# kongqg/marl-sat

Measured on AMD Instinct MI355X. Metric: env-steps/sec (whole node) + MAPPO updates/sec, 4096 envs random 3-SAT, higher is better.
Workload: dtype int32

## Files before the change

marl-sat_amd/csrc/env_kernels.hip:

```cpp
#include <stdlib.h>

#include <algorithm>

#include "common.h"
#include "obs_sparse.h"

namespace msat {

constexpr int kThreads = 256;

struct EnvParams {
    int B, V, C, K, A, M, D;
    int WV, WC;
    int base, rem;
    int max_steps, action_mode, reward_mode, N;
    float r_clause, r_sat, gamma;
    int ablate;
    long long dbg_obs, dbg_assign, dbg_sat, dbg_ntrue, dbg_actions;
    int rq_mode, rq_cap;
    uint32_t rq_serial;
};

struct ObsShadowArg {
    uint32_t *rows;
    int g;
};

enum : int { kModeReset = 0, kModeStep = 1, kModeStepAutoReset = 2, kModeObs = 3 };

__host__ __device__ __forceinline__ uint32_t rq_token(uint32_t serial) { return 0x80000000u | (serial & 0x7FFFFFFFu); }
__host__ __device__ __forceinline__ int rq_capacity(int B) { return (B / 256 + 8 + 7) & ~7; }
__host__ __device__ __forceinline__ size_t rq_words(int B) { return 2 * (size_t)B; }

__device__ __forceinline__ uint32_t *rq_pend(uint32_t *q, int B, int par) { return q + (size_t)par * B; }

__device__ __forceinline__ int rq_scan(const uint32_t *__restrict__ pend, int B, uint32_t tok, int lim, int want,
                                       int *sel) {
    const int lane = threadIdx.x & 63;
    const int W = ((B + 63) / 64 + 3) & ~3;
    const int lo = lane * W;
    int below = 0, mine = 0;
    uint64_t bits = 0;
    for (int i = 0; i < W; i += 4) {
        const int k = lo + i;
        uint4 v = make_uint4(0u, 0u, 0u, 0u);
        if (k < B) v = *reinterpret_cast<const uint4 *>(pend + k);
        const uint32_t w[4] = {v.x, v.y, v.z, v.w};
#pragma unroll
        for (int u = 0; u < 4; ++u) {
            const bool m = k + u < B && w[u] == tok;
            mine += m;
            below += m && k + u < lim;
            if (m && i + u < 64) bits |= 1ull << (i + u);
        }
    }
    int total_below = below;
#pragma unroll
    for (int d = 32; d >= 1; d >>= 1) total_below += __shfl_xor(total_below, d, 64);
    if (want >= 0) {
        int incl = mine;
#pragma unroll
        for (int d = 1; d < 64; d <<= 1) {
            const int up = __shfl_up(incl, d, 64);
            if (lane >= d) incl += up;
        }
        const int excl = incl - mine;
        int found = -1;
        if (want >= excl && want < incl) {
            int r = want - excl;
            if (W <= 64) {
                uint64_t m = bits;
                for (; r > 0; --r) m &= m - 1;
                found = lo + __ffsll((unsigned long long)m) - 1;
            } else {
                for (int i = 0; i < W && found < 0; i += 4) {
                    const int k = lo + i;
                    if (k >= B) break;
                    const uint4 v = *reinterpret_cast<const uint4 *>(pend + k);
                    const uint32_t w[4] = {v.x, v.y, v.z, v.w};
                    for (int u = 0; u < 4 && found < 0; ++u)
                        if (k + u < B && w[u] == tok && r-- == 0) found = k + u;
                }
            }
        }
        const uint64_t has = __ballot(found >= 0);
        *sel = has ? __shfl(found, __ffsll((unsigned long long)has) - 1, 64) : -1;
    }
    return total_below;
}

__host__ __device__ __forceinline__ int agent_lo(const EnvParams &p, int i) { return i * p.base + (i < p.rem ? i : p.rem); }
__host__ __device__ __forceinline__ int agent_size(const EnvParams &p, int i) { return p.base + (i < p.rem ? 1 : 0); }

__device__ __forceinline__ int agent_of_var(const EnvParams &p, int v) {
    const int split = p.rem * (p.base + 1);
    if (v < split) return v / (p.base + 1);
    return p.rem + (v - split) / p.base;
}

struct EnvLds {
    uint32_t *x;
    uint32_t *sat;
    uint32_t *rel;
    uint32_t *nbr;
    uint32_t *fm;
    uint32_t *fx;
    int *red;
    uint32_t *fd;
    uint32_t *sx;
    uint32_t *ssat;
};

__host__ __device__ __forceinline__ int obs_image_words(const EnvParams &p) { return (p.A * p.D) / 32 + 2; }

__host__ __device__ __forceinline__ int shadow_row_words(const EnvParams &p) {
    return 1 + ((p.V + 31) >> 5) + ((p.C + 31) >> 5);
}

__host__ __device__ __forceinline__ size_t env_lds_words(const EnvParams &p, bool sh = false) {
    return (size_t)p.WV + p.WC + (size_t)p.A * (p.WC + p.WV) + 2 * (size_t)obs_image_words(p) + 16 +
           (sh ? (size_t)obs_image_words(p) + 1 + p.WV + p.WC : 0);
}

template <bool SH = false>
__device__ __forceinline__ EnvLds carve(uint32_t *smem, const EnvParams &p) {
    EnvLds l;
    l.x = smem;
    l.sat = l.x + p.WV;
    l.rel = l.sat + p.WC;
    l.nbr = l.rel + (size_t)p.A * p.WC;
    l.fm = l.nbr + (size_t)p.A * p.WV;
    l.fx = l.fm + obs_image_words(p);
    l.fd = l.fx + obs_image_words(p);
    l.sx = l.fd + (SH ? obs_image_words(p) + 1 : 0);
    l.ssat = l.sx + (SH ? p.WV : 0);
    l.red = reinterpret_cast<int *>(l.ssat + (SH ? p.WC : 0));
    return l;
}

__device__ __forceinline__ uint32_t bit(const uint32_t *w, int i) { return (w[i >> 5] >> (i & 31)) & 1u; }

template <int T>
__device__ __forceinline__ void load_x_bits(const EnvParams &p, const EnvLds &l, const uint8_t *__restrict__ xg,
                                            uint32_t x0) {
    const int lane = threadIdx.x & 63;
    for (int v0 = threadIdx.x & ~63; v0 < p.WV * 32; v0 += T) {
        const int v = v0 + lane;
        const uint32_t xv = v0 == (int)(threadIdx.x & ~63) ? x0 : (v < p.V ? xg[v] : 0u);
        const uint64_t m = __ballot(v < p.V && (xv & 1u));
        if (lane < 2) l.x[(v0 >> 5) + lane] = (uint32_t)(m >> (32 * lane));
    }
}
template <int T>
__device__ __forceinline__ void load_x_bits(const EnvParams &p, const EnvLds &l, const uint8_t *__restrict__ xg) {
    load_x_bits<T>(p, l, xg, (int)threadIdx.x < p.V ? xg[threadIdx.x] : 0u);
}

constexpr int kPfClause = 4;
constexpr int kPfRel = 4;
constexpr int kPfNbr = 2;

template <bool kPbrs>
__device__ __forceinline__ void clause_slice(const EnvParams &p, const EnvLds &l, int c0, uint64_t w,
                                             uint8_t *__restrict__ sat_g, uint8_t *__restrict__ ntrue_g, int &unsat,
                                             int &newly) {
    const int lane = threadIdx.x & 63;
    const int c = c0 + lane;
    uint32_t sat = 0, ntrue = 0, old = 0;
    const bool live = c < p.C;
    if (live) {
#pragma unroll
        for (int j = 0; j < 3; ++j) {
            const uint32_t lit = (uint32_t)(w >> (16 * j)) & 0xFFFFu;
            if (lit < MSAT_LIT_ABSENT) ntrue += (bit(l.x, (int)(lit >> 1)) ^ lit) & 1u;
        }
        sat = ntrue ? 1u : 0u;
        if (kPbrs) old = sat_g[c];
        if (sat_g) sat_g[c] = (uint8_t)sat;
        if (ntrue_g) ntrue_g[c] = (uint8_t)ntrue;
    }
    const uint64_t ms = __ballot(sat);
    if (lane < 2) l.sat[(c0 >> 5) + lane] = (uint32_t)(ms >> (32 * lane));
    unsat += __popcll(__ballot(live && !sat));
    if (kPbrs) newly += __popcll(__ballot(sat && !old));
}

template <int T, bool kPbrs, int NPF>
__device__ __forceinline__ void eval_clauses(const EnvParams &p, const EnvLds &l, const uint16_t *__restrict__ lits,
                                             int pidx, uint8_t *__restrict__ sat_g, uint8_t *__restrict__ ntrue_g,
                                             const uint64_t (&pw)[kPfClause]) {
    const uint64_t *prow = reinterpret_cast<const uint64_t *>(lits) + (size_t)pidx * p.C;
    const int lane = threadIdx.x & 63;
    int unsat = 0, newly = 0;
    const int cend = p.WC * 32;
#pragma unroll
    for (int j = 0; j < NPF; ++j) {
        const int c0 = (threadIdx.x & ~63) + j * T;
        if (c0 < cend) clause_slice<kPbrs>(p, l, c0, pw[j], sat_g, ntrue_g, unsat, newly);
    }
    for (int c0 = (threadIdx.x & ~63) + NPF * T; c0 < cend; c0 += T) {
        const int c = c0 + lane;
        const uint64_t w = c < p.C ? prow[c] : 0ull;
        clause_slice<kPbrs>(p, l, c0, w, sat_g, ntrue_g, unsat, newly);
    }
    if (lane == 0) {
        atomicAdd(&l.red[0], unsat);
        if (kPbrs) atomicAdd(&l.red[1], newly);
    }
}


__device__ __forceinline__ uint32_t low_mask(int n) { return n >= 32 ? 0xFFFFFFFFu : ((1u << n) - 1u); }

__device__ __forceinline__ void or_bits(uint32_t *img, int dst, uint32_t bits) {
    if (!bits) return;
    const int w = dst >> 5, s = dst & 31;
    atomicOr(&img[w], bits << s);
    if (s) {
        const uint32_t hi = bits >> (32 - s);
        if (hi) atomicOr(&img[w + 1], hi);
    }
}

template <int T, bool SH>
__device__ __forceinline__ void build_obs_images(const EnvParams &p, const EnvLds &l, bool delta) {
    const int nwV = (p.V + 31) >> 5, nwC = (p.C + 31) >> 5;
    const int U = 2 * nwV + nwC;
    for (int t = threadIdx.x; t < p.A * U; t += T) {
        const int i = t / U;
        int s = t - i * U;
        int len, off;
        uint32_t m, x, xo = 0;
        if (s < nwV) {
            len = min(32, p.V - 32 * s);
            const int lo = agent_lo(p, i) - 32 * s, hi = lo + agent_size(p, i);
            const int a = max(lo, 0), z = min(hi, 32);
            m = z > a ? (low_mask(z) & ~low_mask(a)) : 0u;
            x = l.x[s];
            if (SH && delta) xo = l.sx[s];
            off = 32 * s;
        } else if ((s -= nwV) < nwC) {
            len = min(32, p.C - 32 * s);
            m = l.rel[i * p.WC + s];
            x = l.sat[s];
            if (SH && delta) xo = l.ssat[s];
            off = p.V + 32 * s;
        } else {
            s -= nwC;
            len = min(32, p.V - 32 * s);
            m = l.nbr[i * p.WV + s];
            x = l.x[s];
            if (SH && delta) xo = l.sx[s];
            off = p.V + p.C + 32 * s;
        }
        const uint32_t keep = low_mask(len);
        const int dst = i * p.D + off;
        or_bits(l.fm, dst, m & keep);
        or_bits(l.fx, dst, x & m & keep);
        if (SH && delta) or_bits(l.fd, dst, (x ^ xo) & m & keep);
    }
}

__device__ __forceinline__ uint32_t bits_at(const uint32_t *img, int e) {
    const int w = e >> 5, s = e & 31;
    return (uint32_t)((((uint64_t)img[w + 1] << 32) | img[w]) >> s);
}

__device__ __forceinline__ int elem_val(uint32_t m, uint32_t x, int u) {
    return ((m >> u) & 1u) ? (int)((x >> u) & 1u) : -1;
}

template <typename ObsT>
struct ObsVec;
template <>
struct ObsVec<int32_t> {
    static constexpr int N = 4;
    __device__ static void store(int32_t *dst, uint32_t m, uint32_t x) {
        typedef int v4i __attribute__((ext_vector_type(4)));
        const v4i q = {elem_val(m, x, 0), elem_val(m, x, 1), elem_val(m, x, 2), elem_val(m, x, 3)};
        *reinterpret_cast<v4i *>(dst) = q;
    }
};
template <>
struct ObsVec<int8_t> {
    static constexpr int N = 16;
    __device__ static void store(int8_t *dst, uint32_t m, uint32_t x) {
        typedef unsigned v4u __attribute__((ext_vector_type(4)));
        v4u q;
#pragma unroll
        for (int w = 0; w < 4; ++w) {
            uint32_t word = 0;
#pragma unroll
            for (int u = 0; u < 4; ++u) word |= ((uint32_t)elem_val(m, x, 4 * w + u) & 0xFFu) << (8 * u);
            q[w] = word;
        }
        *reinterpret_cast<v4u *>(dst) = q;
    }
};

template <int T, typename ObsT>
__device__ __forceinline__ void write_obs(const EnvParams &p, const EnvLds &l, ObsT *__restrict__ o) {
    constexpr int VEC = ObsVec<ObsT>::N;
    const int total = p.A * p.D;
    int head = (int)((reinterpret_cast<uintptr_t>(o) / sizeof(ObsT)) % VEC);
    head = head ? VEC - head : 0;
    head = min(head, total);
    for (int e = threadIdx.x; e < head; e += T) o[e] = (ObsT)elem_val(bits_at(l.fm, e), bits_at(l.fx, e), 0);
    const int nchunks = (total - head) / VEC;
    for (int q = threadIdx.x; q < nchunks; q += T) {
        const int e = head + q * VEC;
        ObsVec<ObsT>::store(o + e, bits_at(l.fm, e), bits_at(l.fx, e));
    }
    for (int e = head + nchunks * VEC + threadIdx.x; e < total; e += T)
        o[e] = (ObsT)elem_val(bits_at(l.fm, e), bits_at(l.fx, e), 0);
}

template <typename ObsT>
__device__ __forceinline__ void dcheck_obs_kept(const EnvLds &l, const ObsT *o, int e, int n) {
#ifdef MSAT_DEBUG
    for (int u = 0; u < n; ++u)
        MSAT_DCHECK((int)o[e + u] == elem_val(bits_at(l.fm, e + u), bits_at(l.fx, e + u), 0) ? 0 : -1 - (e + u), 1);
#endif
}

template <int T, typename ObsT>
__device__ __forceinline__ void write_obs_delta(const EnvParams &p, const EnvLds &l, ObsT *__restrict__ o, int G) {
    constexpr int VEC = ObsVec<ObsT>::N;
    const int total = p.A * p.D;
    const uintptr_t a0 = reinterpret_cast<uintptr_t>(o) / sizeof(ObsT);
    const int GE = G / (int)sizeof(ObsT);
    int head = (int)(a0 % VEC);
    head = head ? VEC - head : 0;
    head = min(head, total);
    for (int e = threadIdx.x; e < head; e += T) {
        if (bit(l.fd, e))
            o[e] = (ObsT)elem_val(bits_at(l.fm, e), bits_at(l.fx, e), 0);
        else
            dcheck_obs_kept(l, o, e, 1);
    }
    const int nchunks = (total - head) / VEC;
    for (int q = threadIdx.x; q < nchunks; q += T) {
        const int e = head + q * VEC;
        const int gs = e - (int)((a0 + (uintptr_t)e) & (uintptr_t)(GE - 1));
        const int lo = max(gs, 0), hi = min(gs + GE, total);
        uint32_t any = 0;
        for (int k = lo; k < hi; k += 32) any |= bits_at(l.fd, k) & low_mask(hi - k);
        if (any)
            ObsVec<ObsT>::store(o + e, bits_at(l.fm, e), bits_at(l.fx, e));
        else
            dcheck_obs_kept(l, o, e, VEC);
    }
    for (int e = head + nchunks * VEC + threadIdx.x; e < total; e += T) {
        if (bit(l.fd, e))
            o[e] = (ObsT)elem_val(bits_at(l.fm, e), bits_at(l.fx, e), 0);
        else
            dcheck_obs_kept(l, o, e, 1);
    }
}

__device__ __forceinline__ int xcd_major(int blk, int n, bool off) {
    return (!off && (n & 7) == 0) ? (blk & 7) * (n >> 3) + (blk >> 3) : blk;
}

__device__ __forceinline__ void lds_barrier() { asm volatile("s_waitcnt lgkmcnt(0)\n\ts_barrier" ::: "memory"); }

struct ClockStamp {
    uint64_t *buf = nullptr;
    uint64_t t0 = 0, r0 = 0;
    __device__ __forceinline__ ClockStamp(uint64_t *stamps, int b) {
        if (stamps != nullptr) {
            t0 = __builtin_amdgcn_s_memtime();
            r0 = __builtin_amdgcn_s_memrealtime();
            buf = stamps + 8 * (size_t)b;
        }
    }
    __device__ __forceinline__ void mark(int i) const {
        if (buf == nullptr) return;
        const uint64_t r = __builtin_amdgcn_s_memrealtime();
        if (threadIdx.x == 0) buf[2 + i] = i == 0 ? r0 : r;
    }
    __device__ __forceinline__ void finish() const {
        if (buf == nullptr) return;
        asm volatile("s_waitcnt vmcnt(0)" ::: "memory");
        const uint64_t t1 = __builtin_amdgcn_s_memtime(), r1 = __builtin_amdgcn_s_memrealtime();
        if (threadIdx.x < 4) {
            const int i = threadIdx.x;
            buf[i == 3 ? 7 : i] = i == 0 ? t1 - t0 : i == 1 ? r1 - r0 : i == 2 ? r0 : r1;
        }
    }
};

__host__ __device__ __forceinline__ ObsGeom obs_geom(const EnvParams &p) {
    return ObsGeom{p.V, p.C, p.A, p.D, p.WV, p.WC, p.base, p.rem};
}

template <typename ObsT>
__device__ __forceinline__ void store_sparse_entry(const EnvParams &p, const EnvLds &l, ObsT *__restrict__ o,
                                                   uint32_t entry, int sh) {
    constexpr int VEC = ObsVec<ObsT>::N;
    if (VEC == 4 && (entry & kSparseFast)) {
        ObsVec<ObsT>::store(o + (int)(((entry >> 8) & 0x7FFFFFu) * 4u) - sh, (entry >> 4) & 15u, entry & 15u);
        return;
    }
    const ObsGeom g = obs_geom(p);
    const int total = p.A * p.D, e = (int)entry - sh;
    const int lo = max(e, 0), hi = min(e + VEC, total);
    uint32_t m = 0, x = 0;
    for (int u = lo; u < hi; ++u) {
        const int v = obs_elem(g, l.x, l.sat, l.rel, l.nbr, u);
        m |= (v >= 0 ? 1u : 0u) << (u - e);
        x |= (v > 0 ? 1u : 0u) << (u - e);
    }
    if (lo == e && hi == e + VEC) {
        ObsVec<ObsT>::store(o + e, m, x);
    } else {
        for (int u = lo; u < hi; ++u) o[u] = (ObsT)elem_val(m, x, u - e);
    }
}

#ifndef MSAT_TASK_CARRY
#define MSAT_TASK_CARRY 1
#endif
template <int T, typename ObsT>
__device__ __forceinline__ void write_obs_sparse16(const EnvParams &p, const EnvLds &l, ObsT *__restrict__ o, int sh,
                                                   const ClockStamp *cs) {
    constexpr int VEC = ObsVec<ObsT>::N;
    const ObsGeom g = obs_geom(p);
    const int U = 2 * ((p.V + 31) >> 5) + ((p.C + 31) >> 5);
    constexpr bool kCarry = MSAT_TASK_CARRY && VEC == 4;
    const TaskIdx stride = task_stride(T, U);
    TaskIdx ti = task_first((int)threadIdx.x, U);
    for (int t0 = 0; t0 < p.A * U; t0 += T) {
        int i, s;
        bool live;
        if constexpr (kCarry) {
            i = ti.i, s = ti.s;
            live = i < p.A;
            task_advance(ti, stride, U);
        } else {
            const int t = t0 + (int)threadIdx.x;
            i = t / U, s = t - i * U;
            live = t < p.A * U;
        }
        SparseTask k;
        uint64_t d = 0;
        if (live && sparse_task<VEC>(g, i, s, l.x, l.sat, l.sx, l.ssat, l.rel, l.nbr, sh, k)) d = k.dirty;
        while (d) {
            store_sparse_entry<ObsT>(p, l, o, sparse_entry<VEC>(k, __ffsll((unsigned long long)d) - 1), sh);
            d &= d - 1;
        }
    }
    if (cs) cs->mark(4);
#ifdef MSAT_DEBUG
    const int total = p.A * p.D;
    for (int q = threadIdx.x; q * VEC < total + sh; q += T) {
        const int lo = max(q * VEC - sh, 0), hi = min(q * VEC - sh + VEC, total);
        bool dirty = false;
        for (int e = lo; e < hi; ++e)
            dirty |= obs_elem(g, l.x, l.sat, l.rel, l.nbr, e) != obs_elem(g, l.sx, l.ssat, l.rel, l.nbr, e);
        if (dirty) continue;
        for (int e = lo; e < hi; ++e)
            MSAT_DCHECK((int)o[e] == obs_elem(g, l.x, l.sat, l.rel, l.nbr, e) ? 0 : -1 - e, 1);
    }
#endif
}

template <int T>
__device__ __forceinline__ void prefetch_instance(const EnvParams &p, const msat_pool &pool, int n,
                                                  uint64_t (&w)[kPfClause], uint32_t (&rl)[kPfRel],
                                                  uint32_t (&nb)[kPfNbr]) {
    const int tid = threadIdx.x;
    const uint64_t *prow = reinterpret_cast<const uint64_t *>(pool.lits) + (size_t)n * p.C;
    const uint32_t *rel_g = pool.rel + (size_t)n * p.A * p.WC;
    const uint32_t *nbr_g = pool.nbr + (size_t)n * p.A * p.WV;
    const int nrel = p.A * p.WC, nnbr = p.A * p.WV;
#pragma unroll
    for (int j = 0; j < kPfClause; ++j) {
        const int c = tid + j * T;
        const uint64_t v = prow[min(c, p.C - 1)];
        w[j] = c < p.C ? v : 0ull;
    }
#pragma unroll
    for (int j = 0; j < kPfRel; ++j) {
        const int t = tid + j * T;
        const uint32_t v = rel_g[min(t, nrel - 1)];
        rl[j] = t < nrel ? v : 0u;
    }
#pragma unroll
    for (int j = 0; j < kPfNbr; ++j) {
        const int t = tid + j * T;
        const uint32_t v = nbr_g[min(t, nnbr - 1)];
        nb[j] = t < nnbr ? v : 0u;
    }
}

__device__ __forceinline__ int reset_instance(const EnvParams &p, const int32_t *__restrict__ new_pidx, uint64_t seed,
                                              uint64_t ctr, int b) {
    if (new_pidx != nullptr) return new_pidx[b];
    const uint4 r = reset_rng_block(seed, ctr, (uint32_t)b, 0u);
    return (int)(((uint64_t)r.x * (uint64_t)p.N) >> 32);
}

template <int T>
__device__ __forceinline__ void reset_assignment(const EnvParams &p, const EnvLds &l,
                                                 const uint8_t *__restrict__ new_assign, uint64_t seed, uint64_t ctr,
                                                 int b) {
    if (new_assign != nullptr) {
        load_x_bits<T>(p, l, new_assign + (size_t)b * p.V);
        return;
    }
    for (int t = threadIdx.x; t < p.WV; t += T) {
        const uint4 r = reset_rng_block(seed, ctr, (uint32_t)b, 1u + (uint32_t)(t >> 2));
        const int lane = t & 3;
        uint32_t w = lane == 0 ? r.x : lane == 1 ? r.y : lane == 2 ? r.z : r.w;
        const int hi = p.V - 32 * t;
        if (hi < 32) w &= hi <= 0 ? 0u : ((1u << hi) - 1u);
        l.x[t] = w;
    }
}

template <typename ObsT, int T, bool SH>
__device__ __forceinline__ void stage_and_write_obs(const EnvParams &p, const EnvLds &l, const msat_pool &pool,
                                                    int pidx, bool pf, const uint32_t (&prel)[kPfRel],
                                                    const uint32_t (&pnbr)[kPfNbr], ObsT *__restrict__ o,
                                                    const ClockStamp *cs, uint32_t *__restrict__ srow, bool delta,
                                                    int delta_g, int ndiff) {
    const int tid = threadIdx.x;
    const int nwV = (p.V + 31) >> 5, nwC = (p.C + 31) >> 5;
    if (!SH || (delta && 4 * ndiff > p.V + p.C)) delta = false;
    const bool sparse = SH && delta && delta_g == 16;
    if (SH && srow != nullptr) {
        if (tid == 0) srow[0] = (uint32_t)pidx;
        for (int t = tid; t < nwV + nwC; t += T) srow[1 + t] = t < nwV ? l.x[t] : l.sat[t - nwV];
    }
    {
        const uint32_t *rel_g = pool.rel + (size_t)pidx * p.A * p.WC;
        const uint32_t *nbr_g = pool.nbr + (size_t)pidx * p.A * p.WV;
        int t0r = 0, t0n = 0;
        if (pf) {
#pragma unroll
            for (int j = 0; j < kPfRel; ++j)
                if (tid + j * T < p.A * p.WC) l.rel[tid + j * T] = prel[j];
#pragma unroll
            for (int j = 0; j < kPfNbr; ++j)
                if (tid + j * T < p.A * p.WV) l.nbr[tid + j * T] = pnbr[j];
            t0r = kPfRel * T;
            t0n = kPfNbr * T;
        }
        for (int t = t0r + tid; t < p.A * p.WC; t += T) l.rel[t] = rel_g[t];
        for (int t = t0n + tid; t < p.A * p.WV; t += T) l.nbr[t] = nbr_g[t];
        if (!sparse)
            for (int t = tid; t < (SH && delta ? 3 * obs_image_words(p) + 1 : 2 * obs_image_words(p)); t += T)
                l.fm[t] = 0u;
    }
    lds_barrier();
    if (cs) cs->mark(3);
    if (SH && sparse) {
        write_obs_sparse16<T, ObsT>(p, l, o, (int)((reinterpret_cast<uintptr_t>(o) / sizeof(ObsT)) % ObsVec<ObsT>::N),
                                    cs);
    } else if ((p.ablate & 3) == 0) {
        build_obs_images<T, SH>(p, l, delta);
        lds_barrier();
        if (cs) cs->mark(4);
        if (SH && delta)
            write_obs_delta<T, ObsT>(p, l, o, delta_g);
        else
            write_obs<T, ObsT>(p, l, o);
    } else {
        constexpr int VEC = ObsVec<ObsT>::N;
        const int n = (p.A * p.D) / VEC;
        for (int q = tid; q < n; q += T) ObsVec<ObsT>::store(o + q * VEC, 0u, 0u);
    }
}

template <int MODE, typename ObsT, int T, bool SH = false>
__device__ __forceinline__ void env_run(const EnvParams &p, const msat_pool &pool, const msat_env_state &st,
                                        const int32_t *__restrict__ actions, const uint8_t *__restrict__ reset_mask,
                                        const int32_t *__restrict__ new_pidx, const uint8_t *__restrict__ new_assign,
                                        uint64_t seed, uint64_t ctr, const msat_step_out &out, ObsT *__restrict__ obs,
                                        int b, uint32_t *smem, const ClockStamp &cs,
                                        const ObsShadowArg sa = ObsShadowArg{nullptr, 0}) {
    const EnvLds l = carve<SH>(smem, p);
    const int tid = threadIdx.x;
    if (MODE == kModeReset && reset_mask != nullptr && reset_mask[b] == 0) return;

    uint8_t *__restrict__ xg = st.assign + (size_t)b * p.V;
    uint8_t *__restrict__ sat_g = st.clause_sat + (size_t)b * p.C;
    uint8_t *__restrict__ ntrue_g = st.clause_ntrue ? st.clause_ntrue + (size_t)b * p.C : nullptr;
    if (tid < 16) l.red[tid] = 0;
    const bool rq_fast = MODE == kModeStepAutoReset && p.rq_mode == 1;
    if (MODE != kModeObs && p.rq_mode == 2 && tid == 0) {
        rq_pend(st.reset_queue, p.B, 0)[b] = 0u;
        rq_pend(st.reset_queue, p.B, 1)[b] = 0u;
    }

    bool do_reset = (MODE == kModeReset);
    int ndiff = 0;
    int step0 = 0, u_old = 0, a0 = 0;
    uint32_t x0 = 0;
    bool covered = false;
    if (MODE != kModeReset) {
        if (MODE != kModeObs && p.action_mode == 0) {
            const int32_t *ap = actions + (size_t)b * p.A + min(tid, p.A - 1);
            if (rq_fast && tid == p.A)
                ap = reinterpret_cast<const int32_t *>(rq_pend(st.reset_queue, p.B, p.rq_serial & 1) + b);
            a0 = *ap;
        }
        x0 = xg[min(tid, p.V - 1)];
    }
    const int srw = shadow_row_words(p);
    uint32_t *const srow = SH ? sa.rows + (size_t)b * srw : nullptr;
    uint32_t sh0 = 0;
    if (SH && MODE != kModeReset) sh0 = srow[min(tid, srw - 1)];
    int pidx = st.problem_idx[b];
    if (MODE != kModeReset) {
        step0 = st.step[b];
        u_old = st.num_unsat[b];
    }
    __builtin_amdgcn_sched_barrier(0);
    if (MSAT_DEBUG_BUILD && tid == 0) {
        if (MODE != kModeReset) MSAT_DCHECK(pidx, p.N);
        MSAT_DCHECK((long long)(b + 1) * p.V - 1, p.dbg_assign);
        MSAT_DCHECK((long long)(b + 1) * p.C - 1, p.dbg_sat);
        if (ntrue_g) MSAT_DCHECK((long long)(b + 1) * p.C - 1, p.dbg_ntrue);
        if (obs) MSAT_DCHECK((long long)(b + 1) * p.A * p.D - 1, p.dbg_obs);
        if (MODE == kModeStep || MODE == kModeStepAutoReset)
            MSAT_DCHECK((long long)(b + 1) * p.A * (p.action_mode == 0 ? 1 : p.M) - 1, p.dbg_actions);
    }
    uint64_t pw[kPfClause];
    uint32_t prel[kPfRel], pnbr[kPfNbr];
    if (MODE != kModeReset) {
        prefetch_instance<T>(p, pool, pidx, pw, prel, pnbr);
        __builtin_amdgcn_sched_barrier(0);
        load_x_bits<T>(p, l, xg, x0);
        lds_barrier();
        cs.mark(1);
        if (SH) {
            const int nwV = (p.V + 31) >> 5;
            for (int t = tid; t < srw; t += T) {
                const uint32_t w = t == tid ? sh0 : srow[t];
                if (t == 0)
                    l.red[5] = (int)w;
                else if (t <= nwV)
                    l.sx[t - 1] = w;
                else
                    l.ssat[t - 1 - nwV] = w;
            }
        }
        if (MODE == kModeObs) {
        } else if (p.action_mode == 0) {
            if (rq_fast && tid < 64) {
                const uint32_t tok = rq_token(p.rq_serial);
                int cov = 0;
                if (__builtin_amdgcn_readlane(a0, p.A) == (int)tok) {
                    int unused;
                    cov = rq_scan(rq_pend(st.reset_queue, p.B, p.rq_serial & 1), p.B, tok, b, -1, &unused) < p.rq_cap;
                }
                if (tid == 0) l.red[3] = cov;
            }
            for (int i = tid; i < p.A; i += T) {
                const int a = i == tid ? a0 : actions[(size_t)b * p.A + i];
                const int n = agent_size(p, i);
                if (a >= n) continue;
                int s = a;
                if (s < 0) {
                    s += p.M;
                    if (s < 0) {
                        if (p.reward_mode == MSAT_REWARD_SINGLE_DELTA) continue;
                        s = 0;
                    }
                }
                if (s < n) {
                    const int v = agent_lo(p, i) + s;
                    atomicXor(&l.x[v >> 5], 1u << (v & 31));
                }
            }
        } else {
            for (int t = tid; t < p.A * p.M; t += T) {
                const int i = t / p.M, j = t - (t / p.M) * p.M;
                if (j < agent_size(p, i) && (actions[(size_t)b * p.A * p.M + t] & 1)) {
                    const int v = agent_lo(p, i) + j;
                    atomicXor(&l.x[v >> 5], 1u << (v & 31));
                }
            }
        }
        lds_barrier();
        covered = rq_fast && l.red[3] != 0;
        uint8_t *const scan_sat = covered ? nullptr : sat_g;
        uint8_t *const scan_ntrue = covered ? nullptr : ntrue_g;
        if (MODE != kModeObs && p.reward_mode == MSAT_REWARD_PBRS)
            eval_clauses<T, true, kPfClause>(p, l, pool.lits, pidx, scan_sat, scan_ntrue, pw);
        else
            eval_clauses<T, false, kPfClause>(p, l, pool.lits, pidx, scan_sat, scan_ntrue, pw);
        lds_barrier();
        cs.mark(2);
        const int u_new = MODE != kModeObs ? __builtin_amdgcn_readfirstlane(l.red[0]) : 0;
        const bool solved = (u_new == 0);
        const bool done = solved || (p.reward_mode == MSAT_REWARD_SINGLE_DELTA ? step0 >= p.max_steps
                                                                               : step0 + 1 >= p.max_steps);
        const bool reset_now = (MODE == kModeStepAutoReset) && (done || covered);
        do_reset = reset_now;
        if (SH && !do_reset) {
            const int nwV = (p.V + 31) >> 5, nwC = (p.C + 31) >> 5;
            int n = 0;
            for (int t = tid & 63; t < nwV + nwC; t += 64)
                n += t < nwV ? __popc(l.x[t] ^ l.sx[t]) : __popc(l.sat[t - nwV] ^ l.ssat[t - nwV]);
#pragma unroll
            for (int d = 32; d >= 1; d >>= 1) n += __shfl_xor(n, d, 64);
            ndiff = n;
        }
        if (MODE != kModeObs && tid == 0) {
            float r;
            if (p.reward_mode == MSAT_REWARD_SINGLE_DELTA) {
                const float up = __fdiv_rn((float)u_old, (float)p.C), un = __fdiv_rn((float)u_new, (float)p.C);
                r = __fmul_rn(__fsub_rn(up, un), 10.0f);
                r = __fadd_rn(r, solved ? p.r_sat : 0.0f);
                r = __fadd_rn(r, -0.005f);
            } else if (p.reward_mode == MSAT_REWARD_PBRS) {
                const float pot_new = (float)(-u_new), pot_old = (float)(-u_old);
                const float r_pbrs = __fsub_rn(__fmul_rn(p.gamma, pot_new), pot_old);
                const float r_cl = __fmul_rn((float)l.red[1], p.r_clause);
                r = __fadd_rn(__fadd_rn(r_pbrs, r_cl), solved ? p.r_sat : 0.0f);
            } else {
                r = solved ? 1.0f : 0.0f;
            }
            out.reward[b] = r;
            out.done[b] = done ? 1 : 0;
            out.solved[b] = solved ? 1 : 0;
            if (out.num_unsat) out.num_unsat[b] = u_new;
            if (out.episode_step) out.episode_step[b] = step0 + 1;
            MSAT_DCHECK(covered && !done ? 1 : 0, 1);
            if (!reset_now) {
                st.num_unsat[b] = u_new;
                st.step[b] = step0 + 1;
                st.done[b] = done ? 1 : 0;
            }
            if (rq_fast) {
                const int next_step = reset_now ? 0 : step0 + 1;
                rq_pend(st.reset_queue, p.B, (p.rq_serial + 1) & 1)[b] =
                    next_step + 1 >= p.max_steps ? rq_token(p.rq_serial + 1u) : 0u;
            }
        }
    }

    if (do_reset) {
        if (MODE != kModeReset) lds_barrier();
        pidx = reset_instance(p, new_pidx, seed, ctr, b);
        if (MSAT_DEBUG_BUILD && tid == 0) MSAT_DCHECK(pidx, p.N);
        reset_assignment<T>(p, l, new_assign, seed, ctr, b);
        if (covered) {
            lds_barrier();
            if (tid == 0) {
                st.step[b] = 0;
                st.done[b] = 0;
                st.problem_idx[b] = pidx;
            }
            for (int v = tid; v < p.V; v += T) xg[v] = (uint8_t)bit(l.x, v);
            return;
        }
        if (tid < 2) l.red[tid] = 0;
        lds_barrier();
        eval_clauses<T, false, 0>(p, l, pool.lits, pidx, sat_g, ntrue_g, pw);
        lds_barrier();
        if (tid == 0) {
            st.num_unsat[b] = l.red[0];
            st.step[b] = 0;
            st.done[b] = 0;
            st.problem_idx[b] = pidx;
        }
    }
    if (MODE != kModeObs)
        for (int v = tid; v < p.V; v += T) xg[v] = (uint8_t)bit(l.x, v);
    if ((p.ablate & 3) == 2 || obs == nullptr) return;
    const bool delta = SH && (MODE == kModeStep || MODE == kModeStepAutoReset) && sa.g != 0 && !do_reset &&
                       l.red[5] == pidx;
    stage_and_write_obs<ObsT, T, SH>(p, l, pool, pidx, (MODE != kModeReset) && !do_reset, prel, pnbr,
                                     obs + (size_t)b * p.A * p.D, &cs, srow, delta, sa.g, ndiff);
}

template <typename ObsT, int T, bool SH>
__device__ __forceinline__ void env_side_reset(const EnvParams &p, const msat_pool &pool, const msat_env_state &st,
                                               const int32_t *__restrict__ new_pidx,
                                               const uint8_t *__restrict__ new_assign, uint64_t seed, uint64_t ctr,
                                               ObsT *__restrict__ obs, int j, uint32_t *smem,
                                               const ObsShadowArg sa = ObsShadowArg{nullptr, 0}) {
    const EnvLds l = carve<SH>(smem, p);
    const int tid = threadIdx.x;
    if (tid < 64) {
        int b = -1;
        rq_scan(rq_pend(st.reset_queue, p.B, p.rq_serial & 1), p.B, rq_token(p.rq_serial), 0, j, &b);
        if (tid == 0) l.red[4] = b;
    }
    if (tid < 4) l.red[tid] = 0;
    lds_barrier();
    const int b = l.red[4];
    if (b < 0) return;
    const int pidx = reset_instance(p, new_pidx, seed, ctr, b);
    if (MSAT_DEBUG_BUILD && tid == 0) MSAT_DCHECK(pidx, p.N);
    uint64_t pw[kPfClause];
    uint32_t prel[kPfRel], pnbr[kPfNbr];
    prefetch_instance<T>(p, pool, pidx, pw, prel, pnbr);
    reset_assignment<T>(p, l, new_assign, seed, ctr, b);
    lds_barrier();
    uint8_t *__restrict__ sat_g = st.clause_sat + (size_t)b * p.C;
    uint8_t *__restrict__ ntrue_g = st.clause_ntrue ? st.clause_ntrue + (size_t)b * p.C : nullptr;
    eval_clauses<T, false, kPfClause>(p, l, pool.lits, pidx, sat_g, ntrue_g, pw);
    lds_barrier();
    if (tid == 0) st.num_unsat[b] = l.red[0];
    if ((p.ablate & 3) == 2 || obs == nullptr) return;
    stage_and_write_obs<ObsT, T, SH>(p, l, pool, pidx, true, prel, pnbr, obs + (size_t)b * p.A * p.D, nullptr,
                                     SH ? sa.rows + (size_t)b * shadow_row_words(p) : nullptr, false, 0, 0);
}

template <int MODE, typename ObsT, int T>
__global__ void __launch_bounds__(T)
env_kernel(EnvParams p, msat_pool pool, msat_env_state st, const int32_t *__restrict__ actions,
           const uint8_t *__restrict__ reset_mask, const int32_t *__restrict__ new_pidx,
           const uint8_t *__restrict__ new_assign, uint64_t seed, uint64_t ctr, msat_step_out out,
           ObsT *__restrict__ obs) {
    extern __shared__ __attribute__((aligned(16))) uint32_t smem[];
    const int side = (MODE == kModeStepAutoReset && p.rq_mode == 1) ? p.rq_cap : 0;
    if ((int)blockIdx.x < side) {
        env_side_reset<ObsT, T, false>(p, pool, st, new_pidx, new_assign, seed, ctr, obs, (int)blockIdx.x, smem);
        return;
    }
    const int b = xcd_major((int)blockIdx.x - side, p.B, p.ablate & 4);
    const ClockStamp cs(out.clock_stamps, b);
    env_run<MODE, ObsT, T, false>(p, pool, st, actions, reset_mask, new_pidx, new_assign, seed, ctr, out, obs, b, smem,
                                  cs);
    cs.finish();
}

#ifndef MSAT_SHADOW_W8_MIN_T
#define MSAT_SHADOW_W8_MIN_T 256
#endif
namespace shadow {
template <int MODE, typename ObsT, int T>
__global__ void __launch_bounds__(T) __attribute__((amdgpu_waves_per_eu(T >= MSAT_SHADOW_W8_MIN_T ? 8 : 1, 8)))
env_kernel(EnvParams p, msat_pool pool, msat_env_state st, const int32_t *__restrict__ actions,
           const uint8_t *__restrict__ reset_mask, const int32_t *__restrict__ new_pidx,
           const uint8_t *__restrict__ new_assign, uint64_t seed, uint64_t ctr, msat_step_out out,
           ObsT *__restrict__ obs, uint32_t *__restrict__ shadow_rows, int shadow_g) {
    extern __shared__ __attribute__((aligned(16))) uint32_t smem[];
    const ObsShadowArg sa{shadow_rows, shadow_g};
    const int side = (MODE == kModeStepAutoReset && p.rq_mode == 1) ? p.rq_cap : 0;
    if ((int)blockIdx.x < side) {
        env_side_reset<ObsT, T, true>(p, pool, st, new_pidx, new_assign, seed, ctr, obs, (int)blockIdx.x, smem,
                                      sa);
        return;
    }
    const int b = xcd_major((int)blockIdx.x - side, p.B, p.ablate & 4);
    const ClockStamp cs(out.clock_stamps, b);
    env_run<MODE, ObsT, T, true>(p, pool, st, actions, reset_mask, new_pidx, new_assign, seed, ctr, out, obs, b, smem,
                                 cs, sa);
    cs.finish();
}
}

struct EnvGroup {
    EnvParams p;
    msat_pool pool;
    msat_env_state st;
    const int32_t *actions;
    msat_step_out out;
    void *obs;
    int begin;
    int gid;
};

struct EnvGroups {
    int G, total, ablate;
    EnvGroup g[MSAT_MAX_GROUPS];
};

static_assert(sizeof(EnvGroups) <= 4096, "EnvGroups is passed by value: kernel arguments are limited to 4 KiB");

__host__ __device__ __forceinline__ uint64_t group_seed(int g) { return (uint64_t)g * 0x9E3779B97F4A7C15ull; }

template <int MODE, typename ObsT, int T>
__global__ void __launch_bounds__(T)
env_group_kernel(EnvGroups gs, uint64_t seed, uint64_t ctr) {
    extern __shared__ __attribute__((aligned(16))) uint32_t smem[];
    const int gb = blockIdx.x;
    int g = 0;
#pragma unroll
    for (int k = 1; k < MSAT_MAX_GROUPS; ++k)
        if (k < gs.G && gb >= gs.g[k].begin) g = k;
    const EnvGroup &e = gs.g[g];
    const ClockStamp cs(e.out.clock_stamps, gb - e.begin);
    env_run<MODE, ObsT, T>(e.p, e.pool, e.st, e.actions, nullptr, nullptr, nullptr, seed ^ group_seed(e.gid), ctr, e.out,
                        reinterpret_cast<ObsT *>(e.obs), gb - e.begin, smem, cs);
    cs.finish();
}


__global__ void pool_pack_kernel(const int32_t *__restrict__ lits, int NC, int K, int V,
                                 uint16_t *__restrict__ pool, int32_t *__restrict__ err) {
    const int t = blockIdx.x * blockDim.x + threadIdx.x;
    if (t >= NC) return;
    uint64_t w = 0;
#pragma unroll
    for (int j = 0; j < MSAT_LIT_SLOTS; ++j) {
        uint32_t code = MSAT_LIT_ABSENT;
        if (j < K) {
            const int lit = lits[(size_t)t * K + j];
            if (lit == 0) {
                code = MSAT_LIT_NULL;
            } else {
                const int a = lit < 0 ? -lit : lit;
                if (a > V) {
                    atomicOr(err, 1);
                    code = MSAT_LIT_NULL;
                } else {
                    code = ((uint32_t)(a - 1) << 1) | (lit < 0 ? 1u : 0u);
                }
            }
        }
        w |= (uint64_t)code << (16 * j);
    }
    reinterpret_cast<uint64_t *>(pool)[t] = w;
}

__global__ void __launch_bounds__(kThreads)
agent_tables_kernel(EnvParams p, const uint16_t *__restrict__ lits, uint32_t *__restrict__ rel_g,
                    uint32_t *__restrict__ nbr_g) {
    extern __shared__ __attribute__((aligned(16))) uint32_t smem[];
    uint32_t *rel = smem;
    uint32_t *nbr = rel + (size_t)p.A * p.WC;
    const int n = blockIdx.x;
    for (int t = threadIdx.x; t < p.A * (p.WC + p.WV); t += kThreads) smem[t] = 0u;
    __syncthreads();
    const uint64_t *prow = reinterpret_cast<const uint64_t *>(lits) + (size_t)n * p.C;
    for (int c = threadIdx.x; c < p.C; c += kThreads) {
        const uint64_t w = prow[c];
        int vars[3], ags[3];
        bool nullLit = false;
#pragma unroll
        for (int j = 0; j < 3; ++j) {
            const uint32_t lit = (uint32_t)(w >> (16 * j)) & 0xFFFFu;
            vars[j] = lit < MSAT_LIT_ABSENT ? (int)(lit >> 1) : -1;
            ags[j] = vars[j] >= 0 ? agent_of_var(p, vars[j]) : -1;
            nullLit |= (lit == MSAT_LIT_NULL);
        }
#pragma unroll
        for (int j = 0; j < 3; ++j) {
            if (ags[j] < 0) continue;
            atomicOr(&rel[ags[j] * p.WC + (c >> 5)], 1u << (c & 31));
#pragma unroll
            for (int k = 0; k < 3; ++k) {
                if (k == j || vars[k] < 0 || ags[k] == ags[j]) continue;
                atomicOr(&nbr[ags[j] * p.WV + (vars[k] >> 5)], 1u << (vars[k] & 31));
            }
        }
        if (nullLit && p.rem > 0) {
            for (int i = p.rem; i < p.A; ++i) {
                atomicOr(&rel[i * p.WC + (c >> 5)], 1u << (c & 31));
#pragma unroll
                for (int k = 0; k < 3; ++k) {
                    if (vars[k] < 0 || ags[k] == i) continue;
                    atomicOr(&nbr[i * p.WV + (vars[k] >> 5)], 1u << (vars[k] & 31));
                }
            }
        }
    }
    __syncthreads();
    for (int t = threadIdx.x; t < p.A * p.WC; t += kThreads) rel_g[(size_t)n * p.A * p.WC + t] = rel[t];
    for (int t = threadIdx.x; t < p.A * p.WV; t += kThreads) nbr_g[(size_t)n * p.A * p.WV + t] = nbr[t];
}

__global__ void __launch_bounds__(kThreads)
env_masks_kernel(EnvParams p, msat_pool pool, const int32_t *__restrict__ problem_idx, int32_t *__restrict__ acm,
                 int32_t *__restrict__ anm, int32_t *__restrict__ l2a) {
    const int b = blockIdx.x;
    const int pidx = problem_idx[b];
    const uint32_t *rel = pool.rel + (size_t)pidx * p.A * p.WC;
    const uint32_t *nbr = pool.nbr + (size_t)pidx * p.A * p.WV;
    if (acm)
        for (int t = threadIdx.x; t < p.A * p.C; t += kThreads) {
            const int i = t / p.C, c = t - i * p.C;
            acm[(size_t)b * p.A * p.C + t] = bit(rel + i * p.WC, c) ? 1 : -1;
        }
    if (anm)
        for (int t = threadIdx.x; t < p.A * p.V; t += kThreads) {
            const int i = t / p.V, v = t - i * p.V;
            anm[(size_t)b * p.A * p.V + t] = bit(nbr + i * p.WV, v) ? 1 : -1;
        }
    if (l2a) {
        const uint64_t *prow = reinterpret_cast<const uint64_t *>(pool.lits) + (size_t)pidx * p.C;
        const int last_agent = agent_of_var(p, p.V - 1);
        for (int t = threadIdx.x; t < p.C * p.K; t += kThreads) {
            const int c = t / p.K, j = t - c * p.K;
            const uint32_t lit = (uint32_t)(prow[c] >> (16 * j)) & 0xFFFFu;
            l2a[(size_t)b * p.C * p.K + t] = lit == MSAT_LIT_NULL ? last_agent : agent_of_var(p, (int)(lit >> 1));
        }
    }
}

__global__ void clause_features_kernel(int BC, const uint8_t *__restrict__ sat,
                                       const uint8_t *__restrict__ ntrue, float *__restrict__ f) {
    const int t = blockIdx.x * blockDim.x + threadIdx.x;
    if (t >= BC) return;
    f[3 * (size_t)t + 0] = (float)sat[t];
    f[3 * (size_t)t + 1] = (float)ntrue[t] / 3.0f;
    f[3 * (size_t)t + 2] = 1.0f;
}

__global__ void __launch_bounds__(kThreads)
static_var_features_kernel(const uint16_t *__restrict__ pool, int V, int C, float *__restrict__ f) {
    extern __shared__ __attribute__((aligned(16))) uint32_t smem[];
    int *deg = reinterpret_cast<int *>(smem);
    const int n = blockIdx.x;
    for (int t = threadIdx.x; t < 2 * V; t += kThreads) deg[t] = 0;
    __syncthreads();
    const uint64_t *prow = reinterpret_cast<const uint64_t *>(pool) + (size_t)n * C;
    for (int c = threadIdx.x; c < C; c += kThreads) {
        const uint64_t w = prow[c];
        for (int j = 0; j < 3; ++j) {
            const uint32_t lit = (uint32_t)(w >> (16 * j)) & 0xFFFFu;
            if (lit < MSAT_LIT_ABSENT) atomicAdd(&deg[2 * (lit >> 1) + (lit & 1)], 1);
        }
    }
    __syncthreads();
    for (int v = threadIdx.x; v < V; v += kThreads) {
        float *o = f + ((size_t)n * V + v) * 3;
        o[0] = (float)deg[2 * v] / (float)C;
        o[1] = (float)deg[2 * v + 1] / (float)C;
        o[2] = 0.0f;
    }
}

__global__ void __launch_bounds__(kThreads)
bc_labels_kernel(EnvParams p, const uint16_t *__restrict__ lits, const int32_t *__restrict__ pidx,
                 const uint8_t *__restrict__ assign, float tau, int32_t *__restrict__ labels,
                 int32_t *__restrict__ deltas) {
    extern __shared__ __attribute__((aligned(16))) uint32_t smem[];
    uint32_t *xb = smem;
    int *dl = reinterpret_cast<int *>(smem + p.WV);
    const int b = blockIdx.x, tid = threadIdx.x;
    const uint8_t *xg = assign + (size_t)b * p.V;
    for (int t = tid; t < p.WV; t += kThreads) {
        uint32_t w = 0;
        for (int k = 0; k < 32; ++k) {
            const int v = 32 * t + k;
            if (v < p.V && (xg[v] & 1u)) w |= 1u << k;
        }
        xb[t] = w;
    }
    for (int v = tid; v < p.V; v += kThreads) dl[v] = 0;
    __syncthreads();
    const uint64_t *prow = reinterpret_cast<const uint64_t *>(lits) + (size_t)pidx[b] * p.C;
    for (int c = tid; c < p.C; c += kThreads) {
        const uint64_t w = prow[c];
        int var[MSAT_LIT_SLOTS];
        bool val[MSAT_LIT_SLOTS];
        bool old = false;
#pragma unroll
        for (int j = 0; j < MSAT_LIT_SLOTS; ++j) {
            const uint32_t code = (uint32_t)(w >> (16 * j)) & 0xFFFFu;
            var[j] = code >= MSAT_LIT_ABSENT ? -1 : (int)(code >> 1);
            val[j] = var[j] >= 0 && ((((xb[var[j] >> 5] >> (var[j] & 31)) & 1u) ^ (code & 1u)) != 0u);
            old = old || val[j];
        }
#pragma unroll
        for (int j = 0; j < MSAT_LIT_SLOTS; ++j) {
            const int v = var[j];
            if (v < 0) continue;
            bool dup = false;
#pragma unroll
            for (int k = 0; k < j; ++k) dup = dup || (var[k] == v);
            if (dup) continue;
            bool nw = false;
#pragma unroll
            for (int k = 0; k < MSAT_LIT_SLOTS; ++k) nw = nw || (var[k] >= 0 && (val[k] != (var[k] == v)));
            if (nw != old) atomicAdd(&dl[v], old ? 1 : -1);
        }
    }
    __syncthreads();
    if (deltas)
        for (int v = tid; v < p.V; v += kThreads) deltas[(size_t)b * p.V + v] = dl[v];
    for (int i = tid; i < p.A; i += kThreads) {
        int best = 0, bi = p.M;
        const int lo = agent_lo(p, i), n = agent_size(p, i);
        for (int j = 0; j < n; ++j) {
            const int d = dl[lo + j];
            if (d < best) {
                best = d;
                bi = j;
            }
        }
        labels[(size_t)b * p.A + i] = ((float)best < tau) ? bi : p.M;
    }
}

__global__ void __launch_bounds__(256)
bc_corrupt_kernel(const uint8_t *__restrict__ src, int n_src, const int32_t *__restrict__ src_row, int S, int V,
                  int n, uint64_t seed, uint64_t ctr, uint8_t *__restrict__ dst) {
    const int s = blockIdx.x * blockDim.x + threadIdx.x;
    if (s >= S) return;
    const uint8_t *x = src + (size_t)min(max(src_row[s], 0), n_src - 1) * V;
    uint8_t *y = dst + (size_t)s * V;
    for (int v = 0; v < V; ++v) y[v] = x[v];
    for (int i = 0; i < n; ++i) {
        const int j = V - n + i;
        const uint4 q = philox4x32_10(make_uint4((uint32_t)ctr, (uint32_t)(ctr >> 32), (uint32_t)s, (uint32_t)i),
                                      (uint32_t)seed, (uint32_t)(seed >> 32));
        const int t = (int)mulhi32(q.x, (uint32_t)j + 1u);
        const int pick = y[t] != x[t] ? j : t;
        MSAT_DCHECK(pick, V);
        y[pick] = x[pick] ^ 1u;
    }
}

__global__ void clause_sat_features_kernel(int BC, const uint8_t *__restrict__ sat, float *__restrict__ f) {
// ... 453 lines not shown
```

Measured before the change: 88.24 million.

## Scatter int32 observation deltas directly from clause literals instead of staging rel/nbr

For int32 observations on the shadow-delta path, the observation update now walks changed clauses and variables and writes only the affected entries. It uses prefetched clause literals, a per-variable owner-agent table in LDS, and neighbor masks. This skips staging the rel/nbr matrices into LDS, the barrier that follows, and the per-task sparse scan. The task-carry option in the old sparse writer is also removed. The cost is extra LDS for the owner table and scattered, uncoalesced global stores.

New measurement: 104.1 million (median of 6 runs). 1.18x the previous value.

```diff
diff --git a/marl-sat_amd/csrc/env_kernels.hip b/marl-sat_amd/csrc/env_kernels.hip
--- a/marl-sat_amd/csrc/env_kernels.hip
+++ b/marl-sat_amd/csrc/env_kernels.hip
@@ -109,6 +109,7 @@
     uint32_t *fd;
     uint32_t *sx;
     uint32_t *ssat;
+    uint16_t *own;
 };
 
 __host__ __device__ __forceinline__ int obs_image_words(const EnvParams &p) { return (p.A * p.D) / 32 + 2; }
@@ -119,7 +120,7 @@
 
 __host__ __device__ __forceinline__ size_t env_lds_words(const EnvParams &p, bool sh = false) {
     return (size_t)p.WV + p.WC + (size_t)p.A * (p.WC + p.WV) + 2 * (size_t)obs_image_words(p) + 16 +
-           (sh ? (size_t)obs_image_words(p) + 1 + p.WV + p.WC : 0);
+           (sh ? (size_t)obs_image_words(p) + 1 + p.WV + p.WC + (p.V + 1) / 2 : 0);
 }
 
 template <bool SH = false>
@@ -135,6 +136,7 @@
     l.sx = l.fd + (SH ? obs_image_words(p) + 1 : 0);
     l.ssat = l.sx + (SH ? p.WV : 0);
     l.red = reinterpret_cast<int *>(l.ssat + (SH ? p.WC : 0));
+    l.own = reinterpret_cast<uint16_t *>(l.red + 16);
     return l;
 }
 
@@ -418,30 +420,16 @@
     }
 }
 
-#ifndef MSAT_TASK_CARRY
-#define MSAT_TASK_CARRY 1
-#endif
 template <int T, typename ObsT>
 __device__ __forceinline__ void write_obs_sparse16(const EnvParams &p, const EnvLds &l, ObsT *__restrict__ o, int sh,
                                                    const ClockStamp *cs) {
     constexpr int VEC = ObsVec<ObsT>::N;
     const ObsGeom g = obs_geom(p);
     const int U = 2 * ((p.V + 31) >> 5) + ((p.C + 31) >> 5);
-    constexpr bool kCarry = MSAT_TASK_CARRY && VEC == 4;
-    const TaskIdx stride = task_stride(T, U);
-    TaskIdx ti = task_first((int)threadIdx.x, U);
     for (int t0 = 0; t0 < p.A * U; t0 += T) {
-        int i, s;
-        bool live;
-        if constexpr (kCarry) {
-            i = ti.i, s = ti.s;
-            live = i < p.A;
-            task_advance(ti, stride, U);
-        } else {
-            const int t = t0 + (int)threadIdx.x;
-            i = t / U, s = t - i * U;
-            live = t < p.A * U;
-        }
+        const int t = t0 + (int)threadIdx.x;
+        const int i = t / U, s = t - i * U;
+        const bool live = t < p.A * U;
         SparseTask k;
         uint64_t d = 0;
         if (live && sparse_task<VEC>(g, i, s, l.x, l.sat, l.sx, l.ssat, l.rel, l.nbr, sh, k)) d = k.dirty;
@@ -465,6 +453,68 @@
 #endif
 }
 
+__device__ __forceinline__ void scatter_clause(const EnvParams &p, const EnvLds &l, int c, uint64_t w,
+                                               int32_t *__restrict__ o) {
+    const uint32_t ns = l.sat[c >> 5];
+    if ((((ns ^ l.ssat[c >> 5]) >> (c & 31)) & 1u) == 0) return;
+    const int32_t val = (int32_t)((ns >> (c & 31)) & 1u);
+    const int k = p.V + c;
+    bool null_lit = false;
+#pragma unroll
+    for (int j = 0; j < 3; ++j) {
+        const uint32_t code = (uint32_t)(w >> (16 * j)) & 0xFFFFu;
+        if (code < MSAT_LIT_ABSENT) {
+            const int e = (int)l.own[code >> 1] * p.D + k;
+            MSAT_DCHECK(e, p.A * p.D);
+            o[e] = val;
+        }
+        null_lit |= code == MSAT_LIT_NULL;
+    }
+    if (null_lit && p.rem > 0)
+        for (int i = p.rem; i < p.A; ++i) o[i * p.D + k] = val;
+}
+
+template <int T>
+__device__ __forceinline__ void scatter_obs(const EnvParams &p, const EnvLds &l, const msat_pool &pool, int pidx,
+                                            const uint64_t (&pw)[kPfClause], const uint32_t (&pnbr)[kPfNbr],
+                                            int32_t *__restrict__ o) {
+    const int tid = threadIdx.x;
+    const uint64_t *prow = reinterpret_cast<const uint64_t *>(pool.lits) + (size_t)pidx * p.C;
+#pragma unroll
+    for (int j = 0; j < kPfClause; ++j) {
+        const int c = tid + j * T;
+        if (c < p.C) scatter_clause(p, l, c, pw[j], o);
+    }
+    for (int c = tid + kPfClause * T; c < p.C; c += T) scatter_clause(p, l, c, prow[c], o);
+    for (int v = tid; v < p.V; v += T) {
+        const uint32_t xw = l.x[v >> 5];
+        if (((xw ^ l.sx[v >> 5]) >> (v & 31)) & 1u) {
+            const int e = (int)l.own[v] * p.D + v;
+            MSAT_DCHECK(e, p.A * p.D);
+            o[e] = (int32_t)((xw >> (v & 31)) & 1u);
+        }
+    }
+    const uint32_t *nbr_g = pool.nbr + (size_t)pidx * p.A * p.WV;
+    const int ntask = p.A * p.WV;
+    const TaskIdx stride = task_stride(T, p.WV);
+    TaskIdx ti = task_first(tid, p.WV);
+    auto task = [&](uint32_t m) {
+        const uint32_t xw = l.x[ti.s];
+        uint32_t fd = (xw ^ l.sx[ti.s]) & m;
+        const int e0 = ti.i * p.D + p.V + p.C + 32 * ti.s;
+        while (fd) {
+            const int k = __ffs((int)fd) - 1;
+            MSAT_DCHECK(e0 + k, p.A * p.D);
+            o[e0 + k] = (int32_t)((xw >> k) & 1u);
+            fd &= fd - 1;
+        }
+        task_advance(ti, stride, p.WV);
+    };
+#pragma unroll
+    for (int j = 0; j < kPfNbr; ++j) task(pnbr[j]);
+    for (int t = tid + kPfNbr * T; t < ntask; t += T) task(nbr_g[t]);
+}
+
 template <int T>
 __device__ __forceinline__ void prefetch_instance(const EnvParams &p, const msat_pool &pool, int n,
                                                   uint64_t (&w)[kPfClause], uint32_t (&rl)[kPfRel],
@@ -521,10 +571,10 @@
 
 template <typename ObsT, int T, bool SH>
 __device__ __forceinline__ void stage_and_write_obs(const EnvParams &p, const EnvLds &l, const msat_pool &pool,
-                                                    int pidx, bool pf, const uint32_t (&prel)[kPfRel],
-                                                    const uint32_t (&pnbr)[kPfNbr], ObsT *__restrict__ o,
-                                                    const ClockStamp *cs, uint32_t *__restrict__ srow, bool delta,
-                                                    int delta_g, int ndiff) {
+                                                    int pidx, bool pf, const uint64_t (&pw)[kPfClause],
+                                                    const uint32_t (&prel)[kPfRel], const uint32_t (&pnbr)[kPfNbr],
+                                                    ObsT *__restrict__ o, const ClockStamp *cs,
+                                                    uint32_t *__restrict__ srow, bool delta, int delta_g, int ndiff) {
     const int tid = threadIdx.x;
     const int nwV = (p.V + 31) >> 5, nwC = (p.C + 31) >> 5;
     if (!SH || (delta && 4 * ndiff > p.V + p.C)) delta = false;
@@ -533,6 +583,27 @@
         if (tid == 0) srow[0] = (uint32_t)pidx;
         for (int t = tid; t < nwV + nwC; t += T) srow[1 + t] = t < nwV ? l.x[t] : l.sat[t - nwV];
     }
+    constexpr bool kScatter = SH && sizeof(ObsT) == 4;
+    if constexpr (kScatter) {
+        if (sparse) {
+            if (cs) cs->mark(3);
+            scatter_obs<T>(p, l, pool, pidx, pw, pnbr, reinterpret_cast<int32_t *>(o));
+            if (cs) cs->mark(4);
+#ifdef MSAT_DEBUG
+            const uint32_t *rel_g = pool.rel + (size_t)pidx * p.A * p.WC;
+            const uint32_t *nbr_g = pool.nbr + (size_t)pidx * p.A * p.WV;
+            for (int t = tid; t < p.A * p.WC; t += T) l.rel[t] = rel_g[t];
+            for (int t = tid; t < p.A * p.WV; t += T) l.nbr[t] = nbr_g[t];
+            lds_barrier();
+            const ObsGeom g = obs_geom(p);
+            for (int e = tid; e < p.A * p.D; e += T) {
+                const int nv = obs_elem(g, l.x, l.sat, l.rel, l.nbr, e);
+                if (nv == obs_elem(g, l.sx, l.ssat, l.rel, l.nbr, e)) MSAT_DCHECK((int)o[e] == nv ? 0 : -1 - e, 1);
+            }
+#endif
+            return;
+        }
+    }
     {
         const uint32_t *rel_g = pool.rel + (size_t)pidx * p.A * p.WC;
         const uint32_t *nbr_g = pool.nbr + (size_t)pidx * p.A * p.WV;
@@ -555,7 +626,7 @@
     }
     lds_barrier();
     if (cs) cs->mark(3);
-    if (SH && sparse) {
+    if (SH && !kScatter && sparse) {
         write_obs_sparse16<T, ObsT>(p, l, o, (int)((reinterpret_cast<uintptr_t>(o) / sizeof(ObsT)) % ObsVec<ObsT>::N),
                                     cs);
     } else if ((p.ablate & 3) == 0) {
@@ -632,6 +703,8 @@
     if (MODE != kModeReset) {
         prefetch_instance<T>(p, pool, pidx, pw, prel, pnbr);
         __builtin_amdgcn_sched_barrier(0);
+        if (SH && sizeof(ObsT) == 4 && sa.g == 16 && (MODE == kModeStep || MODE == kModeStepAutoReset))
+            for (int v = tid; v < p.V; v += T) l.own[v] = (uint16_t)agent_of_var(p, v);
         load_x_bits<T>(p, l, xg, x0);
         lds_barrier();
         cs.mark(1);
@@ -774,7 +847,7 @@
     if ((p.ablate & 3) == 2 || obs == nullptr) return;
     const bool delta = SH && (MODE == kModeStep || MODE == kModeStepAutoReset) && sa.g != 0 && !do_reset &&
                        l.red[5] == pidx;
-    stage_and_write_obs<ObsT, T, SH>(p, l, pool, pidx, (MODE != kModeReset) && !do_reset, prel, pnbr,
+    stage_and_write_obs<ObsT, T, SH>(p, l, pool, pidx, (MODE != kModeReset) && !do_reset, pw, prel, pnbr,
                                      obs + (size_t)b * p.A * p.D, &cs, srow, delta, sa.g, ndiff);
 }
 
@@ -808,7 +881,7 @@
     lds_barrier();
     if (tid == 0) st.num_unsat[b] = l.red[0];
     if ((p.ablate & 3) == 2 || obs == nullptr) return;
-    stage_and_write_obs<ObsT, T, SH>(p, l, pool, pidx, true, prel, pnbr, obs + (size_t)b * p.A * p.D, nullptr,
+    stage_and_write_obs<ObsT, T, SH>(p, l, pool, pidx, true, pw, prel, pnbr, obs + (size_t)b * p.A * p.D, nullptr,
                                      SH ? sa.rows + (size_t)b * shadow_row_words(p) : nullptr, false, 0, 0);
 }
 
```
